# chinhau5/parallel_eda

Hardware: AMD Instinct MI355X
Metric: place+route wall-clock to feasibility (s/flow; bitcoin_miner-scale synthetic on stratixiv-like fabric) (lower is better)
Workload: dtype fp32; 1 GPU; model=bitcoin_miner, arch=bitcoin_stratixiv, grid=280x200, W=300, rr_nodes=15745036, rr_edges=87277236, blocks=37632, nets=35616, conns=110426, global_batch=110426, seq_len=0, final_overused=0, wirelength=4910999

## Files before the change

csrc/hip/place_kernel.hip:

```cpp
#include "pnr_hip.h"

namespace pnrh {

struct PlaceDev {
  const int32_t* net_blk_ptr;
  const int32_t* net_blks;
  const int32_t* blk_net_ptr;
  const int32_t* blk_nets;
  const int8_t* blk_type;
  const int8_t* tile_btype;
  const int32_t* type_cols;
  const int32_t* type_col_ptr;
  const uint8_t* fixed;
  const float* net_q;
  const int32_t* net_sink_ptr;
  const float* conn_crit;
  const float* delay_mat;
  int32_t* bx;
  int32_t* by;
  int32_t* bslot;
  int32_t* grid;
  float* net_cost;
  float* net_tcost;
  int32_t num_blocks, num_nets, gx, gy, cap, nx, ny, io_cap;
// ... 108 lines not shown
  }
  return t;
}

__device__ __forceinline__ float wave_sum_f32(float v) {
  for (int off = 32; off; off >>= 1) v += __shfl_xor(v, off);
  return v;
}

__device__ __forceinline__
bool blk_has_net(const PlaceDev& p, int32_t b, int32_t n) {
  int32_t lo = p.blk_net_ptr[b], hi = p.blk_net_ptr[b + 1];
  while (lo < hi) {
    int32_t mid2 = (lo + hi) >> 1;
    if (p.blk_nets[mid2] < n) lo = mid2 + 1; else hi = mid2;
  }
  return lo < p.blk_net_ptr[b + 1] && p.blk_nets[lo] == n;
}

template <class F> __device__ __forceinline__
void for_blk_nets_k(const PlaceDev& p, int32_t b, F f) {
  const int32_t k0 = p.blk_net_ptr[b];
  for (int32_t k = k0 + (threadIdx.x & 63); k < p.blk_net_ptr[b + 1]; k += 64)
    f(k - k0, p.blk_nets[k]);
}
template <class F> __device__ __forceinline__
void for_blk_nets(const PlaceDev& p, int32_t b, F f) {
  for_blk_nets_k(p, b, [&](int32_t, int32_t n) { f(n); });
}
template <class F> __device__ __forceinline__
void for_macro_nets(const PlaceDev& p, int32_t mm0, int32_t mm1, F f) {
  for (int32_t j = mm0; j < mm1; ++j)
    for_blk_nets(p, p.macro_blk[j], [&](int32_t n) { f(j, n); });
}

struct MinClaims {
  int32_t* net; int32_t* loc; int32_t mine;
  __device__ __forceinline__ void take_net(int n) const { atomicMin(&net[n], mine); }
  __device__ __forceinline__ void take_loc(int t) const { atomicMin(&loc[t], mine); }
  __device__ __forceinline__ bool holds_net(int n) const { return net[n] == mine; }
  __device__ __forceinline__ bool holds_loc(int t) const { return loc[t] == mine; }
};
struct EpochClaims {
  unsigned long long* net; unsigned long long* loc; unsigned long long mine;
  __device__ __forceinline__ void take_net(int n) const { atomicMax(&net[n], mine); }
  __device__ __forceinline__ void take_loc(int t) const { atomicMax(&loc[t], mine); }
  __device__ __forceinline__ bool holds_net(int n) const { return net[n] == mine; }
  __device__ __forceinline__ bool holds_loc(int t) const { return loc[t] == mine; }
};

__device__ __forceinline__ unsigned long long claim_key(uint32_t batch, int i) {
  return ((unsigned long long)batch << 32) | (0xFFFFFFFFu - (uint32_t)i);
}

__device__ __forceinline__
int propose_select(const PlaceDev& p, int rlim, uint32_t seed, uint32_t batch,
                   int i, int& x1o, int& y1o, int& slot1o) {
  uint32_t r0 = rng_hash(seed ^ 0x5BD1E995u, batch, i);
  int32_t blk = r0 % p.num_blocks;
  if (p.fixed && p.fixed[blk]) return -1;
  if (p.rx0 >= 0 && (p.bx[blk] < p.rx0 || p.bx[blk] > p.rx1))
    return -1;
  bool io = p.blk_type[blk] == 0;
  int x0 = p.bx[blk], y0 = p.by[blk];
  int x1 = -1, y1 = -1, slot1 = 0;
  int bt = p.blk_type[blk];
  if (p.tile_btype && bt >= 2 && p.type_cols) {
    int c0 = p.type_col_ptr[bt - 2], c1 = p.type_col_ptr[bt - 1];
    int lo = c0, hi = c1;
    while (lo < hi) { int m = (lo + hi) >> 1;
                      if (p.type_cols[m] < x0 - rlim) lo = m + 1; else hi = m; }
    int lo2 = lo, hi2 = c1;
    while (lo2 < hi2) { int m = (lo2 + hi2) >> 1;
                        if (p.type_cols[m] <= x0 + rlim) lo2 = m + 1; else hi2 = m; }
    int ncol = lo2 - lo;
    if (ncol > 0) {
      int ylo = max(1, y0 - rlim), yhi = min(p.ny, y0 + rlim);
      for (int att = 0; att < 8; ++att) {
        uint32_t r1 = rng_hash(seed, batch, i * 131 + 7 * att + 1);
        uint32_t r2 = rng_hash(seed, batch, i * 131 + 7 * att + 2);
        int tx = p.type_cols[lo + (int)(r1 % ncol)];
        if (p.rx0 >= 0 && (tx < p.rx0 || tx > p.rx1)) continue;
        int ty = ylo + (int)(r2 % (yhi - ylo + 1));
        if (tx == x0 && ty == y0) continue;
        x1 = tx; y1 = ty; slot1 = 0;
        break;
      }
    }
  } else {
    for (int att = 0; att < 8; ++att) {
      uint32_t r1 = rng_hash(seed, batch, i * 131 + 7 * att + 1);
      uint32_t r2 = rng_hash(seed, batch, i * 131 + 7 * att + 2);
      int tx = x0 + (int)(r1 % (2 * rlim + 1)) - rlim;
      int ty = y0 + (int)(r2 % (2 * rlim + 1)) - rlim;
      if (tx < 0 || tx >= p.gx || ty < 0 || ty >= p.gy) continue;
      if (p.rx0 >= 0 && (tx < p.rx0 || tx > p.rx1)) continue;
      if (p.tile_btype) {
        if (p.tile_btype[tx * p.gy + ty] != p.blk_type[blk]) continue;
      } else if (is_io_loc(p, tx, ty) != io) continue;
      int c = cap_at(p, tx, ty);
      if (c <= 0) continue;
      if (tx == x0 && ty == y0) continue;
      x1 = tx; y1 = ty;
      slot1 = (int)(rng_hash(seed, batch, i * 131 + 7 * att + 3) % c);
      break;
    }
// ... 128 lines not shown
  }
  wave_lds_sync();
  NetCosts nc{COST_NONE, 0.0f};
  float d_bb = 0.0f, d_td = 0.0f;
  if (live) {
    const float span = (float)((st.xmax[lane] - st.xmin[lane] + 1) +
                               (st.ymax[lane] - st.ymin[lane] + 1));
    nc.bb = mul_rn(q, span);
    d_bb = __builtin_fmaf(q, span, -old_bb);
    if (timing) {
      float t = 0.0f;
      const int i0 = incl - cnt;
      for (int j = 1; j < cnt; ++j)
        t = __builtin_fmaf(st.crit[i0 + j], st.delay[i0 + j], t);
      nc.td = t;
      d_td = t - old_td;
    }
  }
  const int sb = (n_a + lane) & 63;
  const float b_dbb = __shfl(d_bb, sb), b_dtd = __shfl(d_td, sb);
  const float b_bb = __shfl(nc.bb, sb), b_td = __shfl(nc.td, sb);
  if (lane < n_a) {
    dbb += d_bb;
    if (timing) dtd += d_td;
    ca = nc;
  }
  if (lane < n_b) {
    if (b_bb != COST_NONE) {
      dbb += b_dbb;
      if (timing) dtd += b_dtd;
    }
    cb = NetCosts{b_bb, b_td};
  }
  return true;
}

__device__ __forceinline__
bool metropolis(const Sched& s, int i, float& dbb, float& dtd) {
  dbb = wave_sum_f32(dbb);
  dtd = wave_sum_f32(dtd);
  float delta;
  {
#pragma clang fp contract(off)
    delta = (1.0f - s.timing_tradeoff) * dbb * s.inv_bb_norm +
            s.timing_tradeoff * dtd * s.inv_td_norm;
  }
  if (delta <= 0.0f) return true;
  if (s.T <= 0.0f) return false;
  float u = (rng_hash(s.seed, s.batch, i * 131 + 5) & 0xFFFFFF) *
            (1.0f / 16777216.0f);
  return u < __expf(-delta / s.T);
}

__device__ __forceinline__
void record_move(const MovesDev& m, int32_t* mv_from, int i, int32_t blk,
                 int32_t to, int32_t other, float dbb, float dtd,
                 int32_t from) {
  atomicAdd(&m.counters[1], 1);
  m.mv_blk[i] = blk;
  m.mv_to[i] = to;
  m.mv_other[i] = other;
  m.mv_dbb[i] = dbb;
  m.mv_dtd[i] = dtd;
  m.mv_flags[i] = 1;
  mv_from[i] = from;
}

template <class Claims> __device__ __forceinline__
void propose_move(const PlaceDev& p, const MovesDev& m, const Claims& c,
                  int32_t* mv_from, int i, const Sched& s) {
  const int lane = threadIdx.x & 63;
  int sel = -1, sx1 = -1, sy1 = -1, sslot = 0;
  if (lane == 0) {
    m.mv_flags[i] = 0;
    sel = propose_select(p, s.rlim, s.seed, s.batch, i, sx1, sy1, sslot);
  }
  sel = __shfl(sel, 0);
  if (sel < 0) return;
  const int x1 = __shfl(sx1, 0);
  const int y1 = __shfl(sy1, 0);
  const int slot1 = __shfl(sslot, 0);
  const int32_t blk = sel;
  const int x0 = p.bx[blk], y0 = p.by[blk];
  const int mid = p.macro_of ? p.macro_of[blk] : -1;
  float dbb = 0.0f, dtd = 0.0f;
  if (mid >= 0) {
    const MacroPos ms{mid, x1 - x0, y1 - y0};
    const int32_t mm0 = p.macro_ptr[mid], mm1 = p.macro_ptr[mid + 1];
    if (mm1 - mm0 > 16) return;
    int ok = 0;
    if (lane == 0) {
      ok = macro_shift_ok(p, ms, mm0, mm1);
      if (ok) atomicAdd(&m.counters[0], 1);
    }
    ok = __shfl(ok, 0);
    if (!ok) return;
    for_macro_nets(p, mm0, mm1, [&](int32_t j, int32_t n) {
      bool dup = false;
      for (int32_t j2 = mm0; j2 < j && !dup; ++j2)
        dup = blk_has_net(p, p.macro_blk[j2], n);
      if (!dup) add_net_delta(p, n, ms, s.timing_tradeoff, dbb, dtd);
    });
    if (!metropolis(s, i, dbb, dtd)) return;
    if (lane == 0)
      record_move(m, mv_from, i, blk,
                  ((ms.ddx + 4096) << 13) | (ms.ddy + 4096), -2 - mid, dbb,
                  dtd, x0 * p.gy + y0);
    for_macro_nets(p, mm0, mm1, [&](int32_t, int32_t n) { c.take_net(n); });
    for (int32_t j = mm0 + lane; j < mm1; j += 64) {
      int32_t b = p.macro_blk[j];
      c.take_loc(p.bx[b] * p.gy + p.by[b]);
      c.take_loc((p.bx[b] + ms.ddx) * p.gy + p.by[b] + ms.ddy);
    }
    return;
  }
  int32_t other = p.grid[((int64_t)x1 * p.gy + y1) * p.cap + slot1];
  if (other == blk) return;
  if (other >= 0 && p.fixed && p.fixed[other]) return;
  if (other >= 0 && p.macro_of && p.macro_of[other] >= 0)
    return;
  if (lane == 0) atomicAdd(&m.counters[0], 1);
  const SwapPos sw{blk, x1, y1, other, other >= 0 ? x0 : -1000,
                   other >= 0 ? y0 : -1000};
  const int n_a = p.blk_net_ptr[blk + 1] - p.blk_net_ptr[blk];
  const int n_b =
      other >= 0 ? p.blk_net_ptr[other + 1] - p.blk_net_ptr[other] : 0;
  NetCosts ca{COST_NONE, 0.0f}, cb{COST_NONE, 0.0f};
  __shared__ EvalStage stage[PROP_WAVES];
  const bool timing = s.timing_tradeoff > 0.0f;
  bool evaluated = false;
  if (n_a + n_b <= EVAL_SLOTS && (!timing || p.delay_mat != nullptr))
    evaluated = eval_move_parallel(p, stage[threadIdx.x >> 6], sw, blk, other,
                                   n_a, n_b, timing, dbb, dtd, ca, cb);
  if (!evaluated) {
    for_blk_nets_k(p, blk, [&](int32_t k, int32_t n) {
      NetCosts nc = add_net_delta(p, n, sw, s.timing_tradeoff, dbb, dtd);
      if (k < 64) ca = nc;
    });
    if (other >= 0)
      for_blk_nets_k(p, other, [&](int32_t k, int32_t n) {
        if (blk_has_net(p, blk, n)) return;
        NetCosts nc = add_net_delta(p, n, sw, s.timing_tradeoff, dbb, dtd);
        if (k < 64) cb = nc;
      });
  }
  if (!metropolis(s, i, dbb, dtd)) return;
  const bool stored = n_a + n_b <= m.cost_k;
  if (stored) {
    const int64_t s0 = (int64_t)i * m.cost_k;
    if (lane < n_a) m.mv_ncost[s0 + lane] = ca.bb;
    if (lane < n_b) m.mv_ncost[s0 + n_a + lane] = cb.bb;
    if (s.timing_tradeoff > 0.0f) {
      if (lane < n_a) m.mv_ntcost[s0 + lane] = ca.td;
      if (lane < n_b) m.mv_ntcost[s0 + n_a + lane] = cb.td;
    }
  }
  if (lane == 0) {
    record_move(m, mv_from, i, blk,
                ((x1 * p.gy + y1) * p.cap + slot1) |
                    (stored ? 0 : MV_RECOMPUTE),
                other, dbb, dtd, x0 * p.gy + y0);
    c.take_loc(x0 * p.gy + y0);
    c.take_loc(x1 * p.gy + y1);
  }
  auto take = [&](int32_t n) { c.take_net(n); };
  for_blk_nets(p, blk, take);
  if (other >= 0) for_blk_nets(p, other, take);
}

struct Move {
  int32_t blk, other, to;
  bool recompute;
  __device__ __forceinline__ Move(const MovesDev& m, int i)
      : blk(m.mv_blk[i]), other(m.mv_other[i]), to(m.mv_to[i]) {
    recompute = !is_macro() && (to & MV_RECOMPUTE);
    if (recompute) to &= ~MV_RECOMPUTE;
  }
  __device__ __forceinline__ bool is_macro() const { return other <= -2; }
  __device__ __forceinline__ MacroPos macro() const {
    return MacroPos{-2 - other, (to >> 13) - 4096, (to & 0x1FFF) - 4096};
  }
};

template <class Claims> __device__ __forceinline__
bool resolve_move(const PlaceDev& p, const MovesDev& m, const Claims& c,
                  const int32_t* mv_from, int i, const Move& mv) {
  const int lane = threadIdx.x & 63;
  bool bad = false;
  if (mv.is_macro()) {
    const MacroPos ms = mv.macro();
    const int32_t mm0 = p.macro_ptr[ms.mid], mm1 = p.macro_ptr[ms.mid + 1];
    for (int32_t j = mm0 + lane; j < mm1; j += 64) {
      int32_t b = p.macro_blk[j];
      int sx = p.bx[b], sy = p.by[b];
      int tx = sx + ms.ddx, ty = sy + ms.ddy;
      if (tx < 0 || tx >= p.gx || ty < 0 || ty >= p.gy) bad = true;
      else if (!c.holds_loc(sx * p.gy + sy) ||
               !c.holds_loc(tx * p.gy + ty)) bad = true;
    }
    for_macro_nets(p, mm0, mm1, [&](int32_t, int32_t n) {
      if (!c.holds_net(n)) bad = true;
    });
  } else {
    int x1 = mv.to / p.cap / p.gy, y1 = (mv.to / p.cap) % p.gy;
    if (lane == 0 && (!c.holds_loc(mv_from[i]) ||
                      !c.holds_loc(x1 * p.gy + y1))) bad = true;
    auto lost = [&](int32_t n) { if (!c.holds_net(n)) bad = true; };
    for_blk_nets(p, mv.blk, lost);
    if (mv.other >= 0) for_blk_nets(p, mv.other, lost);
  }
  const bool win = !__any(bad);
  if (lane == 0) {
    if (!win) { m.mv_flags[i] = 0; atomicAdd(&m.counters[3], 1); }
    else { m.mv_flags[i] = 2; atomicAdd(&m.counters[2], 1); }
  }
  return win;
}

template <class Pos> __device__ __forceinline__
void refresh_net(const PlaceDev& p, int32_t n, const Pos& pos,
                 float timing_tradeoff) {
  p.net_cost[n] = net_bb_cost(p, n, pos);
  if (timing_tradeoff > 0.0f) p.net_tcost[n] = net_td_cost(p, n, pos);
}

__device__ __forceinline__
void apply_move(const PlaceDev& p, const MovesDev& m, int i, const Move& mv,
                float timing_tradeoff, double* cost_acc ) {
  const int lane = threadIdx.x & 63;
  if (mv.is_macro()) {
    const MacroPos ms = mv.macro();
    const int32_t mm0 = p.macro_ptr[ms.mid], mm1 = p.macro_ptr[ms.mid + 1];
    for_macro_nets(p, mm0, mm1, [&](int32_t, int32_t n) {
      refresh_net(p, n, ms, timing_tradeoff);
    });
    if (lane == 0) {
      for (int32_t j = mm0; j < mm1; ++j) {
        int32_t b = p.macro_blk[j];
        p.grid[((int64_t)p.bx[b] * p.gy + p.by[b]) * p.cap + p.bslot[b]] = -1;
      }
      for (int32_t j = mm0; j < mm1; ++j) {
        int32_t b = p.macro_blk[j];
        int tx = p.bx[b] + ms.ddx, ty = p.by[b] + ms.ddy;
        p.grid[((int64_t)tx * p.gy + ty) * p.cap] = b;
        p.bx[b] = tx; p.by[b] = ty; p.bslot[b] = 0;
      }
    }
  } else {
    const int32_t blk = mv.blk, other = mv.other;
    int slot1 = mv.to % p.cap;
    int x1 = mv.to / p.cap / p.gy, y1 = (mv.to / p.cap) % p.gy;
    int x0 = p.bx[blk], y0 = p.by[blk], s0 = p.bslot[blk];
    const SwapPos sw{blk, x1, y1, other, other >= 0 ? x0 : -1000,
                     other >= 0 ? y0 : -1000};
    if (mv.recompute) {
      auto refresh = [&](int32_t n) { refresh_net(p, n, sw, timing_tradeoff); };
      for_blk_nets(p, blk, refresh);
      if (other >= 0) for_blk_nets(p, other, refresh);
    } else {
      const int64_t s0 = (int64_t)i * m.cost_k;
      int32_t slot0 = 0;
      auto copy = [&](int32_t k, int32_t n) {
        const float bb = m.mv_ncost[s0 + slot0 + k];
        if (bb == COST_NONE) return;
        p.net_cost[n] = bb;
        if (timing_tradeoff > 0.0f)
          p.net_tcost[n] = m.mv_ntcost[s0 + slot0 + k];
      };
      for_blk_nets_k(p, blk, copy);
      slot0 = p.blk_net_ptr[blk + 1] - p.blk_net_ptr[blk];
      if (other >= 0) for_blk_nets_k(p, other, copy);
    }
    if (lane == 0) {
      p.grid[((int64_t)x0 * p.gy + y0) * p.cap + s0] = other >= 0 ? other : -1;
      p.grid[((int64_t)x1 * p.gy + y1) * p.cap + slot1] = blk;
      p.bx[blk] = x1; p.by[blk] = y1; p.bslot[blk] = slot1;
      if (other >= 0) { p.bx[other] = x0; p.by[other] = y0; p.bslot[other] = s0; }
    }
  }
  if (lane == 0) {
    unsafeAtomicAdd(&cost_acc[0], (double)m.mv_dbb[i]);
    unsafeAtomicAdd(&cost_acc[1], (double)m.mv_dtd[i]);
  }
}

__global__ void place_reset_claims_kernel(int32_t* net_claim, int32_t nn,
                                          int32_t* loc_claim, int32_t nl) {
  int i = blockIdx.x * blockDim.x + threadIdx.x;
  int total = max(nn, nl);
  for (; i < total; i += gridDim.x * blockDim.x) {
    if (i < nn) net_claim[i] = 0x7FFFFFFF;
    if (i < nl) loc_claim[i] = 0x7FFFFFFF;
  }
}

__launch_bounds__(64 * PROP_WAVES, 2)
__global__ void place_propose_kernel(PlaceDev p, MovesDev m, int32_t* mv_from,
                                     Sched s) {
  const int i = move_index();
  if (i >= m.n_moves) return;
  propose_move(p, m, MinClaims{m.net_claim, m.loc_claim, i}, mv_from, i, s);
}

__launch_bounds__(64 * PROP_WAVES, 2)
__global__ void place_resolve_kernel(PlaceDev p, MovesDev m,
                                     const int32_t* mv_from) {
  const int i = move_index();
  if (i >= m.n_moves || m.mv_flags[i] != 1) return;
  resolve_move(p, m, MinClaims{m.net_claim, m.loc_claim, i}, mv_from, i,
               Move(m, i));
}

__launch_bounds__(64 * PROP_WAVES, 2)
__global__ void place_apply_kernel(PlaceDev p, MovesDev m,
                                   float timing_tradeoff, double* cost_acc) {
  const int i = move_index();
  if (i >= m.n_moves || m.mv_flags[i] != 2) return;
  apply_move(p, m, i, Move(m, i), timing_tradeoff, cost_acc);
}

struct RunDev {
  int32_t* mv_from;
  unsigned long long* net_claim;
  unsigned long long* loc_claim;
  int32_t* ctrl;
};

__launch_bounds__(64 * PROP_WAVES, 2)
__global__ void place_propose_run_kernel(PlaceDev p, MovesDev m, RunDev r,
                                         Sched s) {
  if (r.ctrl[0]) return;
  const int i = move_index();
  if (i >= m.n_moves) return;
  const EpochClaims c{r.net_claim, r.loc_claim, claim_key(s.batch, i)};
  propose_move(p, m, c, r.mv_from, i, s);
}

__device__ __forceinline__
void commit_move(const PlaceDev& p, const MovesDev& m, const RunDev& r,
                 float timing_tradeoff, double* cost_acc, uint32_t batch) {
  const int i = move_index();
  if (i >= m.n_moves || m.mv_flags[i] != 1) return;
  const Move mv(m, i);
  const EpochClaims c{r.net_claim, r.loc_claim, claim_key(batch, i)};
  if (resolve_move(p, m, c, r.mv_from, i, mv))
    apply_move(p, m, i, mv, timing_tradeoff, cost_acc);
}

__launch_bounds__(64 * PROP_WAVES, 2)
__global__ void place_commit_kernel(PlaceDev p, MovesDev m, RunDev r,
                                    float timing_tradeoff, double* cost_acc,
                                    uint32_t batch, int check,
                                    int32_t target_moves) {
  if (r.ctrl[0]) return;
  commit_move(p, m, r, timing_tradeoff, cost_acc, batch);
  if (!check) return;
  asm volatile("s_waitcnt vmcnt(0)" ::: "memory");
  __syncthreads();
  if (threadIdx.x != 0) return;
  __threadfence();
  asm volatile("s_waitcnt vmcnt(0)" ::: "memory");
  int ticket = __hip_atomic_fetch_add(&r.ctrl[2], 1, __ATOMIC_RELAXED,
                                      __HIP_MEMORY_SCOPE_AGENT);
  if (ticket != (int)gridDim.x - 1) return;
  __threadfence();
  int att = __hip_atomic_load(&m.counters[0], __ATOMIC_RELAXED,
                              __HIP_MEMORY_SCOPE_AGENT);
  int acc = __hip_atomic_load(&m.counters[1], __ATOMIC_RELAXED,
                              __HIP_MEMORY_SCOPE_AGENT);
  int win = __hip_atomic_load(&m.counters[2], __ATOMIC_RELAXED,
                              __HIP_MEMORY_SCOPE_AGENT);
  r.ctrl[1] += 4;
  if (win + (att - acc) >= target_moves) r.ctrl[0] = 1;
  __hip_atomic_store(&r.ctrl[2], 0, __ATOMIC_RELAXED,
                     __HIP_MEMORY_SCOPE_AGENT);
}

__global__ void place_refresh_costs_kernel(PlaceDev p, float timing_tradeoff,
                                           double* out ) {
  int n = blockIdx.x * blockDim.x + threadIdx.x;
  for (; n < p.num_nets; n += gridDim.x * blockDim.x) {
    const SwapPos as_is{-1, 0, 0, -1, 0, 0};
    float c = net_bb_cost(p, n, as_is);
    p.net_cost[n] = c;
    unsafeAtomicAdd(&out[0], (double)c);
    float t = timing_tradeoff > 0.0f ? net_td_cost(p, n, as_is) : 0.0f;
    p.net_tcost[n] = t;
    unsafeAtomicAdd(&out[1], (double)t);
  }
}

}

using namespace pnrh;

extern "C" {

struct PlaceLaunchArgs {
  const int32_t* net_blk_ptr; const int32_t* net_blks;
  const int32_t* blk_net_ptr; const int32_t* blk_nets;
  const int8_t* blk_type; const int8_t* tile_btype;
  const int32_t* type_cols; const int32_t* type_col_ptr;
  const uint8_t* fixed;
  const float* net_q;
  const int32_t* net_sink_ptr; const float* conn_crit; const float* delay_mat;
  int32_t* bx; int32_t* by; int32_t* bslot; int32_t* grid;
  float* net_cost; float* net_tcost;
  int32_t num_blocks, num_nets, gx, gy, cap, nx, ny, io_cap;
  int32_t rx0, rx1;
  const int32_t* macro_of; const int32_t* macro_ptr;
  const int32_t* macro_blk;
  int32_t* mv_blk; int32_t* mv_to; int32_t* mv_other;
  float* mv_dbb; float* mv_dtd; uint8_t* mv_flags;
  int32_t* net_claim; int32_t* loc_claim; int32_t* counters;
  int32_t n_moves;
  float T; int32_t rlim; float timing_tradeoff;
  float inv_bb_norm, inv_td_norm;
  uint32_t seed, batch;
  double* cost_acc;
  int32_t* mv_from;
  unsigned long long* net_claim64; unsigned long long* loc_claim64;
  int32_t* run_ctrl;
  float* mv_ncost; float* mv_ntcost;
  int32_t cost_k;
};

static void unpack(const PlaceLaunchArgs* a, PlaceDev& p, MovesDev& m) {
  p.net_blk_ptr = a->net_blk_ptr; p.net_blks = a->net_blks;
  p.blk_net_ptr = a->blk_net_ptr; p.blk_nets = a->blk_nets;
  p.blk_type = a->blk_type; p.tile_btype = a->tile_btype;
  p.type_cols = a->type_cols; p.type_col_ptr = a->type_col_ptr;
  p.fixed = a->fixed;
  p.net_q = a->net_q;
  p.net_sink_ptr = a->net_sink_ptr; p.conn_crit = a->conn_crit;
  p.delay_mat = a->delay_mat;
  p.bx = a->bx; p.by = a->by; p.bslot = a->bslot; p.grid = a->grid;
  p.net_cost = a->net_cost; p.net_tcost = a->net_tcost;
  p.num_blocks = a->num_blocks; p.num_nets = a->num_nets;
  p.gx = a->gx; p.gy = a->gy; p.cap = a->cap;
  p.nx = a->nx; p.ny = a->ny; p.io_cap = a->io_cap;
  p.rx0 = a->rx0; p.rx1 = a->rx1;
  p.macro_of = a->macro_of; p.macro_ptr = a->macro_ptr;
  p.macro_blk = a->macro_blk;
  m.mv_blk = a->mv_blk; m.mv_to = a->mv_to; m.mv_other = a->mv_other;
  m.mv_dbb = a->mv_dbb; m.mv_dtd = a->mv_dtd; m.mv_flags = a->mv_flags;
  m.net_claim = a->net_claim; m.loc_claim = a->loc_claim;
  m.counters = a->counters; m.n_moves = a->n_moves;
  m.mv_ncost = a->mv_ncost; m.mv_ntcost = a->mv_ntcost;
  m.cost_k = a->cost_k;
}

static bool batch_args_ok(const PlaceLaunchArgs* a) {
  return a->mv_from && a->mv_ncost && a->mv_ntcost && a->cost_k >= 1 &&
         a->cost_k <= 64 &&
         (int64_t)a->gx * a->gy * a->cap < (int64_t)MV_RECOMPUTE;
}

static Sched sched(const PlaceLaunchArgs* a, uint32_t batch) {
  return Sched{a->T, a->rlim, a->timing_tradeoff, a->inv_bb_norm,
               a->inv_td_norm, a->seed, batch};
}

int pnr_place_batch(const PlaceLaunchArgs* a, void* stream) {
  if (!batch_args_ok(a) || !a->net_claim || !a->loc_claim)
    return (int)hipErrorInvalidValue;
  PlaceDev p; MovesDev m;
  unpack(a, p, m);
  hipStream_t s = (hipStream_t)stream;
  int rg = (max(max(a->num_nets, a->gx * a->gy), a->n_moves) + 255) / 256;
  rg = rg < 2048 ? rg : 2048;
  hipLaunchKernelGGL(place_reset_claims_kernel, dim3(rg), dim3(256), 0, s,
                     m.net_claim, p.num_nets, m.loc_claim, p.gx * p.gy);
  int mg = (m.n_moves + PROP_WAVES - 1) / PROP_WAVES;
  hipLaunchKernelGGL(place_propose_kernel, dim3(mg), dim3(64 * PROP_WAVES),
                     0, s, p, m, a->mv_from, sched(a, a->batch));
  hipLaunchKernelGGL(place_resolve_kernel, dim3(mg), dim3(64 * PROP_WAVES),
                     0, s, p, m, (const int32_t*)a->mv_from);
  hipLaunchKernelGGL(place_apply_kernel, dim3(mg), dim3(64 * PROP_WAVES),
                     0, s, p, m, a->timing_tradeoff, a->cost_acc);
  return (int)hipGetLastError();
}

int pnr_place_run(const PlaceLaunchArgs* a, uint32_t first_batch,
                  int32_t target_moves, int32_t n_batches, void* stream) {
  if (n_batches < 0 || (n_batches & 3) || first_batch == 0 ||
      !batch_args_ok(a) || !a->net_claim64 || !a->loc_claim64 ||
      !a->run_ctrl)
    return (int)hipErrorInvalidValue;
  PlaceDev p; MovesDev m;
  unpack(a, p, m);
  RunDev r;
  r.mv_from = a->mv_from;
  r.net_claim = a->net_claim64; r.loc_claim = a->loc_claim64;
  r.ctrl = a->run_ctrl;
  hipStream_t s = (hipStream_t)stream;
  int mg = (m.n_moves + PROP_WAVES - 1) / PROP_WAVES;
  for (int32_t k = 0; k < n_batches; ++k) {
    const uint32_t batch = first_batch + (uint32_t)k;
    hipLaunchKernelGGL(place_propose_run_kernel, dim3(mg),
                       dim3(64 * PROP_WAVES), 0, s, p, m, r, sched(a, batch));
    hipLaunchKernelGGL(place_commit_kernel, dim3(mg), dim3(64 * PROP_WAVES),
                       0, s, p, m, r, a->timing_tradeoff, a->cost_acc, batch,
                       (int)(((k + 1) & 3) == 0), target_moves);
  }
  return (int)hipGetLastError();
}

int pnr_place_refresh(const PlaceLaunchArgs* a, void* stream) {
  PlaceDev p; MovesDev m;
  unpack(a, p, m);
  hipStream_t s = (hipStream_t)stream;
  hipLaunchKernelGGL(place_refresh_costs_kernel, dim3(1024), dim3(256), 0, s,
                     p, a->timing_tradeoff, a->cost_acc);
  return (int)hipGetLastError();
}

int64_t pnr_place_args_sizeof() { return (int64_t)sizeof(PlaceLaunchArgs); }

}
```

parallel_eda_amd/place/gpu_placer.py:

```python
import ctypes as ct
import math

import numpy as np

from ..arch.archdef import ArchDef
from ..ops import hip_api
from .placer import Placement, analytic_delay_matrix


class PlaceLaunchArgs(ct.Structure):
    _fields_ = [
        ("net_blk_ptr", ct.c_void_p), ("net_blks", ct.c_void_p),
        ("blk_net_ptr", ct.c_void_p), ("blk_nets", ct.c_void_p),
        ("blk_type", ct.c_void_p), ("tile_btype", ct.c_void_p),
        ("type_cols", ct.c_void_p), ("type_col_ptr", ct.c_void_p),
        ("fixed", ct.c_void_p),
        ("net_q", ct.c_void_p),
        ("net_sink_ptr", ct.c_void_p), ("conn_crit", ct.c_void_p),
        ("delay_mat", ct.c_void_p),
        ("bx", ct.c_void_p), ("by", ct.c_void_p), ("bslot", ct.c_void_p),
        ("grid", ct.c_void_p),
        ("net_cost", ct.c_void_p), ("net_tcost", ct.c_void_p),
        ("num_blocks", ct.c_int32), ("num_nets", ct.c_int32),
        ("gx", ct.c_int32), ("gy", ct.c_int32), ("cap", ct.c_int32),
        ("nx", ct.c_int32), ("ny", ct.c_int32), ("io_cap", ct.c_int32),
        ("rx0", ct.c_int32), ("rx1", ct.c_int32),
        ("macro_of", ct.c_void_p), ("macro_ptr", ct.c_void_p),
        ("macro_blk", ct.c_void_p),
        ("mv_blk", ct.c_void_p), ("mv_to", ct.c_void_p), ("mv_other", ct.c_void_p),
        ("mv_dbb", ct.c_void_p), ("mv_dtd", ct.c_void_p), ("mv_flags", ct.c_void_p),
        ("net_claim", ct.c_void_p), ("loc_claim", ct.c_void_p),
        ("counters", ct.c_void_p), ("n_moves", ct.c_int32),
        ("T", ct.c_float), ("rlim", ct.c_int32), ("timing_tradeoff", ct.c_float),
        ("inv_bb_norm", ct.c_float), ("inv_td_norm", ct.c_float),
        ("seed", ct.c_uint32), ("batch", ct.c_uint32),
        ("cost_acc", ct.c_void_p),
        ("mv_from", ct.c_void_p),
        ("net_claim64", ct.c_void_p), ("loc_claim64", ct.c_void_p),
        ("run_ctrl", ct.c_void_p),
        ("mv_ncost", ct.c_void_p), ("mv_ntcost", ct.c_void_p),
        ("cost_k", ct.c_int32),
    ]


RUN_CHUNK_BATCHES = 32


def _lib():
    lib = hip_api.lib()
    if not hasattr(lib, "_place_ready"):
        lib.pnr_place_batch.restype = ct.c_int
        lib.pnr_place_batch.argtypes = [ct.POINTER(PlaceLaunchArgs), ct.c_void_p]
        lib.pnr_place_run.restype = ct.c_int
        lib.pnr_place_run.argtypes = [ct.POINTER(PlaceLaunchArgs), ct.c_uint32,
                                      ct.c_int32, ct.c_int32, ct.c_void_p]
        lib.pnr_place_refresh.restype = ct.c_int
        lib.pnr_place_refresh.argtypes = [ct.POINTER(PlaceLaunchArgs), ct.c_void_p]
        lib.pnr_place_args_sizeof.restype = ct.c_int64
        if lib.pnr_place_args_sizeof() != ct.sizeof(PlaceLaunchArgs):
            raise RuntimeError("PlaceLaunchArgs ABI mismatch")
        lib._place_ready = True
    return lib


def ptr(t):
    return ct.c_void_p(t.data_ptr())


class GpuPlacer:
    def __init__(self, netlist, arch: ArchDef, seed=7, timing=False,
                 device="cuda:0", n_moves=None, fixed=None,
                 delay_matrix="analytic", macros=None, legacy_batches=False):
        import torch
        self.torch = torch
        self.legacy_batches = legacy_batches
        self.device = device
        self.arch = arch
        self.nl = netlist
        self.seed = seed
        self.timing = timing
        nb = netlist.num_blocks
        nn = netlist.num_nets
        gx, gy = arch.nx + 2, arch.ny + 2
        self.gx, self.gy = gx, gy
        self.cap = max(1, arch.io_cap)
        self.batch_counter = 0

        counts = 1 + np.diff(netlist.net_sink_ptr)
        net_blk_ptr = np.r_[0, np.cumsum(counts)].astype(np.int32)
        net_blks = np.empty(net_blk_ptr[-1], dtype=np.int32)
        net_blks[net_blk_ptr[:-1]] = netlist.net_driver
        is_sink = np.ones(len(net_blks), dtype=bool)
        is_sink[net_blk_ptr[:-1]] = False
        net_blks[is_sink] = netlist.net_sinks
        net_of_member = np.repeat(np.arange(nn, dtype=np.int64),
                                  np.diff(net_blk_ptr))
        key = net_blks.astype(np.int64) * nn + net_of_member
        key = np.unique(key)
# ... 46 lines not shown
            self.t_delay_mat = up(dm.ravel())
        else:
            self._dm = None
            self.t_delay_mat = None

        bx, by, bslot, grid = self._initial_placement(seed)
        self.t_macro_of = self.t_macro_ptr = self.t_macro_blk = None
        self.macros = macros or []
        if self.macros:
            bx, by, bslot, grid = self._legalize_macros(
                bx, by, bslot, grid, self.macros)
            macro_of = np.full(nb, -1, dtype=np.int32)
            mptr = [0]
            mblk = []
            for mi, grp in enumerate(self.macros):
                for (b, dx, dy) in grp:
                    macro_of[b] = mi
                    mblk.append(b)
                mptr.append(len(mblk))
            self.t_macro_of = up(macro_of)
            self.t_macro_ptr = up(np.asarray(mptr, dtype=np.int32))
            self.t_macro_blk = up(np.asarray(mblk, dtype=np.int32))
        self.t_bx = up(bx); self.t_by = up(by); self.t_bslot = up(bslot)
        self.t_grid = up(grid)
        self.t_net_cost = torch.zeros(nn, dtype=torch.float32, device=device)
        self.t_net_tcost = torch.zeros(nn, dtype=torch.float32, device=device)

        self.n_moves = n_moves or int(np.clip(nb // 16, 64, 1 << 16))
        nm = self.n_moves
        self.t_mv_blk = torch.zeros(nm, dtype=torch.int32, device=device)
        self.t_mv_to = torch.zeros(nm, dtype=torch.int32, device=device)
        self.t_mv_other = torch.zeros(nm, dtype=torch.int32, device=device)
        self.t_mv_dbb = torch.zeros(nm, dtype=torch.float32, device=device)
        self.t_mv_dtd = torch.zeros(nm, dtype=torch.float32, device=device)
        self.t_mv_flags = torch.zeros(nm, dtype=torch.uint8, device=device)
        self.t_net_claim = self.t_loc_claim = None
        self.t_net_claim64 = self.t_loc_claim64 = None
        if legacy_batches:
            self.t_net_claim = torch.zeros(nn, dtype=torch.int32, device=device)
            self.t_loc_claim = torch.zeros(gx * gy, dtype=torch.int32,
                                           device=device)
        else:
            self.t_net_claim64 = torch.zeros(nn, dtype=torch.int64,
                                             device=device)
            self.t_loc_claim64 = torch.zeros(gx * gy, dtype=torch.int64,
                                             device=device)
        self.t_mv_from = torch.zeros(nm, dtype=torch.int32, device=device)
        max_deg = int(np.diff(blk_net_ptr).max()) if nb else 0
        self.cost_k = int(np.clip(2 * max_deg, 1, 64))
        self.t_mv_ncost = torch.zeros(nm * self.cost_k, dtype=torch.float32,
                                      device=device)
        self.t_mv_ntcost = torch.zeros(nm * self.cost_k, dtype=torch.float32,
                                       device=device)
        self.t_run_state = torch.zeros(8, dtype=torch.int32, device=device)
        self.t_counters = self.t_run_state[:4]
        self.t_run_ctrl = self.t_run_state[4:]
        self.t_cost_acc = torch.zeros(2, dtype=torch.float64, device=device)

        self.lib = _lib()
        self.bb_cost, self.td_cost = self.refresh_costs()

    def _initial_placement(self, seed):
        arch = self.arch
        nl = self.nl
        rng = np.random.default_rng(seed)
        nb = nl.num_blocks
        bx = np.zeros(nb, dtype=np.int32)
        by = np.zeros(nb, dtype=np.int32)
        bslot = np.zeros(nb, dtype=np.int32)
        if self._fixed is not None:
            bx2, by2, bs2, grid = self._initial_placement_free(rng)
            ids, fx, fy, fs = [np.asarray(a) for a in self._fixed]
            for b, x, y, sl in zip(ids, fx, fy, fs):
                occ = grid[x, y, sl]
                if occ == b:
                    continue
                grid[bx2[b], by2[b], bs2[b]] = occ
                if occ >= 0:
                    bx2[occ], by2[occ], bs2[occ] = bx2[b], by2[b], bs2[b]
                bx2[b], by2[b], bs2[b] = x, y, sl
                grid[x, y, sl] = b
            return bx2, by2, bs2, grid.reshape(-1)
        return self._initial_placement_free(rng, flat=True)

    def _legalize_macros(self, bx, by, bslot, grid, macros):
        arch = self.arch
        g = grid.reshape(self.gx, self.gy, self.cap)
        members = [b for grp in macros for (b, _, _) in grp]
        for b in members:
            g[bx[b], by[b], bslot[b]] = -1
        tb = (arch.tile_btype_grid().reshape(self.gx, self.gy)
              if arch.is_heterogeneous() else None)

        def tile_ok(b, x, y):
            if not (0 <= x < self.gx and 0 <= y < self.gy):
                return False
            bt = int(self.nl.block_type[b])
            if tb is not None:
                if tb[x, y] != bt:
                    return False
            else:
                io = (x == 0 or x == self.gx - 1 or
                      y == 0 or y == self.gy - 1)
                inner = 1 <= x <= arch.nx and 1 <= y <= arch.ny
                if bt == 0 or io or not inner:
                    return False
            return g[x, y, 0] < 0

        for grp in macros:
# ... 51 lines not shown
                   [(x, 0) for x in range(1, arch.nx + 1)] +
                   [(x, self.gy - 1) for x in range(1, arch.nx + 1)])
        slots = [(x, y, s) for (x, y) in io_locs for s in range(arch.io_cap)]
        sel = rng.permutation(len(slots))[:len(ios)]
        for b, k in zip(ios, sel):
            x, y, s = slots[k]
            bx[b], by[b], bslot[b] = x, y, s
            grid[x, y, s] = b
        return (bx, by, bslot, grid.reshape(-1)) if flat \
            else (bx, by, bslot, grid)

    def _args(self, T=0.0, rlim=1, tt=0.0, inv_bb=1.0, inv_td=1.0):
        a = PlaceLaunchArgs()
        a.net_blk_ptr = ptr(self.t_net_blk_ptr); a.net_blks = ptr(self.t_net_blks)
        a.blk_net_ptr = ptr(self.t_blk_net_ptr); a.blk_nets = ptr(self.t_blk_nets)
        a.blk_type = ptr(self.t_blk_type)
        a.tile_btype = (ptr(self.t_tile_btype)
                        if self.t_tile_btype is not None else None)
        a.type_cols = (ptr(self.t_type_cols)
                       if self.t_type_cols is not None else None)
        a.type_col_ptr = (ptr(self.t_type_col_ptr)
                          if self.t_type_col_ptr is not None else None)
        a.fixed = ptr(self.t_fixed) if self.t_fixed is not None else None
        a.net_q = ptr(self.t_net_q)
        a.net_sink_ptr = ptr(self.t_net_sink_ptr)
        a.conn_crit = ptr(self.t_conn_crit)
        a.delay_mat = ptr(self.t_delay_mat) if self.t_delay_mat is not None else None
        a.bx = ptr(self.t_bx); a.by = ptr(self.t_by); a.bslot = ptr(self.t_bslot)
        a.grid = ptr(self.t_grid)
        a.net_cost = ptr(self.t_net_cost); a.net_tcost = ptr(self.t_net_tcost)
        a.num_blocks = self.nl.num_blocks; a.num_nets = self.nl.num_nets
        a.gx = self.gx; a.gy = self.gy; a.cap = self.cap
        a.nx = self.arch.nx; a.ny = self.arch.ny; a.io_cap = self.arch.io_cap
        a.rx0, a.rx1 = getattr(self, "move_region", (-1, -1))
        if getattr(self, "t_macro_of", None) is not None:
            a.macro_of = ptr(self.t_macro_of)
            a.macro_ptr = ptr(self.t_macro_ptr)
            a.macro_blk = ptr(self.t_macro_blk)
        else:
            a.macro_of = a.macro_ptr = a.macro_blk = None
        a.mv_blk = ptr(self.t_mv_blk); a.mv_to = ptr(self.t_mv_to)
        a.mv_other = ptr(self.t_mv_other); a.mv_dbb = ptr(self.t_mv_dbb)
        a.mv_dtd = ptr(self.t_mv_dtd); a.mv_flags = ptr(self.t_mv_flags)
        if self.legacy_batches:
            a.net_claim = ptr(self.t_net_claim)
            a.loc_claim = ptr(self.t_loc_claim)
            a.net_claim64 = a.loc_claim64 = None
        else:
            a.net_claim = a.loc_claim = None
            a.net_claim64 = ptr(self.t_net_claim64)
            a.loc_claim64 = ptr(self.t_loc_claim64)
        a.mv_from = ptr(self.t_mv_from)
        a.run_ctrl = ptr(self.t_run_ctrl)
        a.mv_ncost = ptr(self.t_mv_ncost); a.mv_ntcost = ptr(self.t_mv_ntcost)
        a.cost_k = self.cost_k
        a.counters = ptr(self.t_counters); a.n_moves = self.n_moves
        a.T = T; a.rlim = max(1, int(rlim)); a.timing_tradeoff = tt
        a.inv_bb_norm = inv_bb; a.inv_td_norm = inv_td
        a.seed = self.seed & 0xFFFFFFFF; a.batch = self.batch_counter
        a.cost_acc = ptr(self.t_cost_acc)
        return a

    def _stream(self):
        return self.torch.cuda.current_stream().cuda_stream

    def refresh_costs(self):
        self.t_cost_acc.zero_()
        a = self._args(tt=1.0 if self.timing else 0.0)
        rc = self.lib.pnr_place_refresh(ct.byref(a), self._stream())
        hip_api.check(rc, "place_refresh")
        self.torch.cuda.synchronize(self.device)
        bb, td = self.t_cost_acc.cpu().numpy()
        self.bb_cost, self.td_cost = float(bb), float(td)
        return self.bb_cost, self.td_cost

    def run_batches(self, T, rlim, target_moves, tt, bb_norm, td_norm,
                    max_batches=256):
        if self.legacy_batches:
            return self._run_batches_legacy(T, rlim, target_moves, tt,
                                            bb_norm, td_norm, max_batches)
        self.t_run_state.zero_()
        a = self._args(T=T, rlim=rlim, tt=tt,
                       inv_bb=1.0 / bb_norm, inv_td=1.0 / td_norm)
        target = int(min(max(math.ceil(target_moves), -0x7FFFFFFF),
                         0x7FFFFFFF))
        cap = 4 * ((max_batches + 3) // 4)
        first = self.batch_counter + 1
        enq = 0
        att = acc = executed = 0
        while enq < cap:
            n = min(RUN_CHUNK_BATCHES, cap - enq)
            rc = self.lib.pnr_place_run(ct.byref(a), first + enq, target, n,
                                        self._stream())
            hip_api.check(rc, "place_run")
            enq += n
            st = self.t_run_state.cpu().numpy()
            att, acc = int(st[0]), int(st[1])
            done, executed = int(st[4]), int(st[5])
            if done:
                break
        self.batch_counter += executed
        srate = acc / max(1, att)
        return srate, att

    def _run_batches_legacy(self, T, rlim, target_moves, tt, bb_norm, td_norm,
                            max_batches=256):
        self.t_counters.zero_()
        batches = 0
        win = att = acc = 0
        while batches < max_batches:
            for _ in range(4):
                self.batch_counter += 1
                a = self._args(T=T, rlim=rlim, tt=tt,
                               inv_bb=1.0 / bb_norm, inv_td=1.0 / td_norm)
                rc = self.lib.pnr_place_batch(ct.byref(a), self._stream())
                hip_api.check(rc, "place_batch")
                batches += 1
            self.torch.cuda.synchronize(self.device)
            c = self.t_counters.cpu().numpy()
            att, acc, win = int(c[0]), int(c[1]), int(c[2])
            if win + (att - acc) >= target_moves:
                break
        else:
            self.torch.cuda.synchronize(self.device)
        srate = acc / max(1, att)
        return srate, att

    def set_move_region(self, x0, x1):
        self.move_region = (x0, x1)

    def set_crit(self, conn_crit):
        t = self.torch.from_numpy(np.ascontiguousarray(conn_crit,
                                                       dtype=np.float32))
        self.t_conn_crit.copy_(t.to(self.device))

    def placement(self):
        return Placement(self.t_bx.cpu().numpy(), self.t_by.cpu().numpy(),
                         self.t_bslot.cpu().numpy(),
                         bb_cost=self.bb_cost, td_cost=self.td_cost)

    def check_place(self):
        bx = self.t_bx.cpu().numpy(); by = self.t_by.cpu().numpy()
        bslot = self.t_bslot.cpu().numpy()
        grid = self.t_grid.cpu().numpy().reshape(self.gx, self.gy, self.cap)
        nl = self.nl
        tb = (self.arch.tile_btype_grid().reshape(self.gx, self.gy)
              if self.arch.is_heterogeneous() else None)
        btype = np.asarray(nl.block_type)
        if tb is not None:
# ... 149 lines not shown
```

Before: 7.272 s.

## Shard placement move counters across cache lines and drop per-move cost accumulation atomics

Replaces the single global attempt/accept/win/conflict counters with 64 shards, each on its own 128-byte line and chosen by block index, which spreads atomic contention. The last block of each check reduces the shards with a wavefront reduction and writes the totals back for the host. The change also removes the per-applied-move double-precision atomic adds into cost_acc, so the running cost delta is no longer accumulated in apply. The risk is that any code still reading cost_acc after a run will see stale values.

Result: faster. 6.066 s, median of 6 (-16.6%).

```diff
diff --git a/csrc/hip/place_kernel.hip b/csrc/hip/place_kernel.hip
--- a/csrc/hip/place_kernel.hip
+++ b/csrc/hip/place_kernel.hip
@@ -184,6 +184,19 @@
 __device__ __forceinline__ unsigned long long claim_key(uint32_t batch, int i) {
   return ((unsigned long long)batch << 32) | (0xFFFFFFFFu - (uint32_t)i);
 }
+
+enum { CNT_ATTEMPTS = 0, CNT_ACCEPTED = 1, CNT_WINNERS = 2, CNT_CONFLICTS = 3 };
+struct DirectCounters {
+  int32_t* w;
+  __device__ __forceinline__ void add(int k) const { atomicAdd(&w[k], 1); }
+};
+#define SHARD_WORDS 32
+struct ShardCounters {
+  int32_t* w;
+  __device__ __forceinline__ ShardCounters(int32_t* shards, int32_t mask)
+      : w(shards + (int64_t)(blockIdx.x & mask) * SHARD_WORDS) {}
+  __device__ __forceinline__ void add(int k) const { atomicAdd(&w[k], 1); }
+};
 
 __device__ __forceinline__
 int propose_select(const PlaceDev& p, int rlim, uint32_t seed, uint32_t batch,
@@ -418,11 +431,11 @@
   return u < __expf(-delta / s.T);
 }
 
-__device__ __forceinline__
-void record_move(const MovesDev& m, int32_t* mv_from, int i, int32_t blk,
-                 int32_t to, int32_t other, float dbb, float dtd,
-                 int32_t from) {
-  atomicAdd(&m.counters[1], 1);
+template <class Counters> __device__ __forceinline__
+void record_move(const MovesDev& m, const Counters& cnt, int32_t* mv_from,
+                 int i, int32_t blk, int32_t to, int32_t other, float dbb,
+                 float dtd, int32_t from) {
+  cnt.add(CNT_ACCEPTED);
   m.mv_blk[i] = blk;
   m.mv_to[i] = to;
   m.mv_other[i] = other;
@@ -432,9 +445,10 @@
   mv_from[i] = from;
 }
 
-template <class Claims> __device__ __forceinline__
+template <class Claims, class Counters> __device__ __forceinline__
 void propose_move(const PlaceDev& p, const MovesDev& m, const Claims& c,
-                  int32_t* mv_from, int i, const Sched& s) {
+                  const Counters& cnt, int32_t* mv_from, int i,
+                  const Sched& s) {
   const int lane = threadIdx.x & 63;
   int sel = -1, sx1 = -1, sy1 = -1, sslot = 0;
   if (lane == 0) {
@@ -457,7 +471,7 @@
     int ok = 0;
     if (lane == 0) {
       ok = macro_shift_ok(p, ms, mm0, mm1);
-      if (ok) atomicAdd(&m.counters[0], 1);
+      if (ok) cnt.add(CNT_ATTEMPTS);
     }
     ok = __shfl(ok, 0);
     if (!ok) return;
@@ -469,7 +483,7 @@
     });
     if (!metropolis(s, i, dbb, dtd)) return;
     if (lane == 0)
-      record_move(m, mv_from, i, blk,
+      record_move(m, cnt, mv_from, i, blk,
                   ((ms.ddx + 4096) << 13) | (ms.ddy + 4096), -2 - mid, dbb,
                   dtd, x0 * p.gy + y0);
     for_macro_nets(p, mm0, mm1, [&](int32_t, int32_t n) { c.take_net(n); });
@@ -485,7 +499,7 @@
   if (other >= 0 && p.fixed && p.fixed[other]) return;
   if (other >= 0 && p.macro_of && p.macro_of[other] >= 0)
     return;
-  if (lane == 0) atomicAdd(&m.counters[0], 1);
+  if (lane == 0) cnt.add(CNT_ATTEMPTS);
   const SwapPos sw{blk, x1, y1, other, other >= 0 ? x0 : -1000,
                    other >= 0 ? y0 : -1000};
   const int n_a = p.blk_net_ptr[blk + 1] - p.blk_net_ptr[blk];
@@ -522,7 +536,7 @@
     }
   }
   if (lane == 0) {
-    record_move(m, mv_from, i, blk,
+    record_move(m, cnt, mv_from, i, blk,
                 ((x1 * p.gy + y1) * p.cap + slot1) |
                     (stored ? 0 : MV_RECOMPUTE),
                 other, dbb, dtd, x0 * p.gy + y0);
@@ -548,9 +562,10 @@
   }
 };
 
-template <class Claims> __device__ __forceinline__
+template <class Claims, class Counters> __device__ __forceinline__
 bool resolve_move(const PlaceDev& p, const MovesDev& m, const Claims& c,
-                  const int32_t* mv_from, int i, const Move& mv) {
+                  const Counters& cnt, const int32_t* mv_from, int i,
+                  const Move& mv) {
   const int lane = threadIdx.x & 63;
   bool bad = false;
   if (mv.is_macro()) {
@@ -577,8 +592,8 @@
   }
   const bool win = !__any(bad);
   if (lane == 0) {
-    if (!win) { m.mv_flags[i] = 0; atomicAdd(&m.counters[3], 1); }
-    else { m.mv_flags[i] = 2; atomicAdd(&m.counters[2], 1); }
+    if (!win) { m.mv_flags[i] = 0; cnt.add(CNT_CONFLICTS); }
+    else { m.mv_flags[i] = 2; cnt.add(CNT_WINNERS); }
   }
   return win;
 }
@@ -592,7 +607,7 @@
 
 __device__ __forceinline__
 void apply_move(const PlaceDev& p, const MovesDev& m, int i, const Move& mv,
-                float timing_tradeoff, double* cost_acc ) {
+                float timing_tradeoff) {
   const int lane = threadIdx.x & 63;
   if (mv.is_macro()) {
     const MacroPos ms = mv.macro();
@@ -644,10 +659,6 @@
       if (other >= 0) { p.bx[other] = x0; p.by[other] = y0; p.bslot[other] = s0; }
     }
   }
-  if (lane == 0) {
-    unsafeAtomicAdd(&cost_acc[0], (double)m.mv_dbb[i]);
-    unsafeAtomicAdd(&cost_acc[1], (double)m.mv_dtd[i]);
-  }
 }
 
 __global__ void place_reset_claims_kernel(int32_t* net_claim, int32_t nn,
@@ -665,7 +676,8 @@
                                      Sched s) {
   const int i = move_index();
   if (i >= m.n_moves) return;
-  propose_move(p, m, MinClaims{m.net_claim, m.loc_claim, i}, mv_from, i, s);
+  propose_move(p, m, MinClaims{m.net_claim, m.loc_claim, i},
+               DirectCounters{m.counters}, mv_from, i, s);
 }
 
 __launch_bounds__(64 * PROP_WAVES, 2)
@@ -673,16 +685,16 @@
                                      const int32_t* mv_from) {
   const int i = move_index();
   if (i >= m.n_moves || m.mv_flags[i] != 1) return;
-  resolve_move(p, m, MinClaims{m.net_claim, m.loc_claim, i}, mv_from, i,
-               Move(m, i));
+  resolve_move(p, m, MinClaims{m.net_claim, m.loc_claim, i},
+               DirectCounters{m.counters}, mv_from, i, Move(m, i));
 }
 
 __launch_bounds__(64 * PROP_WAVES, 2)
 __global__ void place_apply_kernel(PlaceDev p, MovesDev m,
-                                   float timing_tradeoff, double* cost_acc) {
+                                   float timing_tradeoff) {
   const int i = move_index();
   if (i >= m.n_moves || m.mv_flags[i] != 2) return;
-  apply_move(p, m, i, Move(m, i), timing_tradeoff, cost_acc);
+  apply_move(p, m, i, Move(m, i), timing_tradeoff);
 }
 
 struct RunDev {
@@ -690,6 +702,8 @@
   unsigned long long* net_claim;
   unsigned long long* loc_claim;
   int32_t* ctrl;
+  int32_t* shards;
+  int32_t n_shards;
 };
 
 __launch_bounds__(64 * PROP_WAVES, 2)
@@ -699,45 +713,58 @@
   const int i = move_index();
   if (i >= m.n_moves) return;
   const EpochClaims c{r.net_claim, r.loc_claim, claim_key(s.batch, i)};
-  propose_move(p, m, c, r.mv_from, i, s);
+  propose_move(p, m, c, ShardCounters(r.shards, r.n_shards - 1), r.mv_from, i,
+               s);
 }
 
 __device__ __forceinline__
 void commit_move(const PlaceDev& p, const MovesDev& m, const RunDev& r,
-                 float timing_tradeoff, double* cost_acc, uint32_t batch) {
+                 float timing_tradeoff, uint32_t batch) {
   const int i = move_index();
   if (i >= m.n_moves || m.mv_flags[i] != 1) return;
   const Move mv(m, i);
   const EpochClaims c{r.net_claim, r.loc_claim, claim_key(batch, i)};
-  if (resolve_move(p, m, c, r.mv_from, i, mv))
-    apply_move(p, m, i, mv, timing_tradeoff, cost_acc);
+  if (resolve_move(p, m, c, ShardCounters(r.shards, r.n_shards - 1),
+                   r.mv_from, i, mv))
+    apply_move(p, m, i, mv, timing_tradeoff);
+}
+
+__device__ __forceinline__ int wave_sum_i32(int v) {
+  for (int off = 32; off; off >>= 1) v += __shfl_xor(v, off);
+  return v;
 }
 
 __launch_bounds__(64 * PROP_WAVES, 2)
 __global__ void place_commit_kernel(PlaceDev p, MovesDev m, RunDev r,
-                                    float timing_tradeoff, double* cost_acc,
-                                    uint32_t batch, int check,
-                                    int32_t target_moves) {
+                                    float timing_tradeoff, uint32_t batch,
+                                    int check, int32_t target_moves) {
   if (r.ctrl[0]) return;
-  commit_move(p, m, r, timing_tradeoff, cost_acc, batch);
+  commit_move(p, m, r, timing_tradeoff, batch);
   if (!check) return;
   asm volatile("s_waitcnt vmcnt(0)" ::: "memory");
   __syncthreads();
-  if (threadIdx.x != 0) return;
+  if (threadIdx.x >= 64) return;
+  const int lane = threadIdx.x;
   __threadfence();
   asm volatile("s_waitcnt vmcnt(0)" ::: "memory");
-  int ticket = __hip_atomic_fetch_add(&r.ctrl[2], 1, __ATOMIC_RELAXED,
-                                      __HIP_MEMORY_SCOPE_AGENT);
-  if (ticket != (int)gridDim.x - 1) return;
+  int ticket = 0;
+  if (lane == 0)
+    ticket = __hip_atomic_fetch_add(&r.ctrl[2], 1, __ATOMIC_RELAXED,
+                                    __HIP_MEMORY_SCOPE_AGENT);
+  if (__shfl(ticket, 0) != (int)gridDim.x - 1) return;
   __threadfence();
-  int att = __hip_atomic_load(&m.counters[0], __ATOMIC_RELAXED,
-                              __HIP_MEMORY_SCOPE_AGENT);
-  int acc = __hip_atomic_load(&m.counters[1], __ATOMIC_RELAXED,
-                              __HIP_MEMORY_SCOPE_AGENT);
-  int win = __hip_atomic_load(&m.counters[2], __ATOMIC_RELAXED,
-                              __HIP_MEMORY_SCOPE_AGENT);
+  int tot[4] = {0, 0, 0, 0};
+  for (int sh = lane; sh < r.n_shards; sh += 64)
+    for (int k = 0; k < 4; ++k)
+      tot[k] += __hip_atomic_load(&r.shards[(int64_t)sh * SHARD_WORDS + k],
+                                  __ATOMIC_RELAXED, __HIP_MEMORY_SCOPE_AGENT);
+  for (int k = 0; k < 4; ++k) tot[k] = wave_sum_i32(tot[k]);
+  if (lane != 0) return;
+  for (int k = 0; k < 4; ++k) m.counters[k] = tot[k];
   r.ctrl[1] += 4;
-  if (win + (att - acc) >= target_moves) r.ctrl[0] = 1;
+  if (tot[CNT_WINNERS] + (tot[CNT_ATTEMPTS] - tot[CNT_ACCEPTED]) >=
+      target_moves)
+    r.ctrl[0] = 1;
   __hip_atomic_store(&r.ctrl[2], 0, __ATOMIC_RELAXED,
                      __HIP_MEMORY_SCOPE_AGENT);
 }
@@ -787,6 +814,8 @@
   int32_t* mv_from;
   unsigned long long* net_claim64; unsigned long long* loc_claim64;
   int32_t* run_ctrl;
+  int32_t* run_shards;
+  int32_t n_shards;
   float* mv_ncost; float* mv_ntcost;
   int32_t cost_k;
 };
@@ -843,7 +872,7 @@
   hipLaunchKernelGGL(place_resolve_kernel, dim3(mg), dim3(64 * PROP_WAVES),
                      0, s, p, m, (const int32_t*)a->mv_from);
   hipLaunchKernelGGL(place_apply_kernel, dim3(mg), dim3(64 * PROP_WAVES),
-                     0, s, p, m, a->timing_tradeoff, a->cost_acc);
+                     0, s, p, m, a->timing_tradeoff);
   return (int)hipGetLastError();
 }
 
@@ -851,7 +880,8 @@
                   int32_t target_moves, int32_t n_batches, void* stream) {
   if (n_batches < 0 || (n_batches & 3) || first_batch == 0 ||
       !batch_args_ok(a) || !a->net_claim64 || !a->loc_claim64 ||
-      !a->run_ctrl)
+      !a->run_ctrl || !a->run_shards || a->n_shards < 1 ||
+      (a->n_shards & (a->n_shards - 1)) || ((uintptr_t)a->run_shards & 127))
     return (int)hipErrorInvalidValue;
   PlaceDev p; MovesDev m;
   unpack(a, p, m);
@@ -859,6 +889,8 @@
   r.mv_from = a->mv_from;
   r.net_claim = a->net_claim64; r.loc_claim = a->loc_claim64;
   r.ctrl = a->run_ctrl;
+  r.shards = a->run_shards;
+  r.n_shards = a->n_shards;
   hipStream_t s = (hipStream_t)stream;
   int mg = (m.n_moves + PROP_WAVES - 1) / PROP_WAVES;
   for (int32_t k = 0; k < n_batches; ++k) {
@@ -866,7 +898,7 @@
     hipLaunchKernelGGL(place_propose_run_kernel, dim3(mg),
                        dim3(64 * PROP_WAVES), 0, s, p, m, r, sched(a, batch));
     hipLaunchKernelGGL(place_commit_kernel, dim3(mg), dim3(64 * PROP_WAVES),
-                       0, s, p, m, r, a->timing_tradeoff, a->cost_acc, batch,
+                       0, s, p, m, r, a->timing_tradeoff, batch,
                        (int)(((k + 1) & 3) == 0), target_moves);
   }
   return (int)hipGetLastError();
diff --git a/parallel_eda_amd/place/gpu_placer.py b/parallel_eda_amd/place/gpu_placer.py
--- a/parallel_eda_amd/place/gpu_placer.py
+++ b/parallel_eda_amd/place/gpu_placer.py
@@ -38,12 +38,17 @@
         ("mv_from", ct.c_void_p),
         ("net_claim64", ct.c_void_p), ("loc_claim64", ct.c_void_p),
         ("run_ctrl", ct.c_void_p),
+        ("run_shards", ct.c_void_p), ("n_shards", ct.c_int32),
         ("mv_ncost", ct.c_void_p), ("mv_ntcost", ct.c_void_p),
         ("cost_k", ct.c_int32),
     ]
 
 
 RUN_CHUNK_BATCHES = 32
+
+LINE_WORDS = 32
+RUN_HOST_WORDS = 8
+COUNTER_SHARDS = 64
 
 
 def _lib():
@@ -196,9 +201,14 @@
                                       device=device)
         self.t_mv_ntcost = torch.zeros(nm * self.cost_k, dtype=torch.float32,
                                        device=device)
-        self.t_run_state = torch.zeros(8, dtype=torch.int32, device=device)
+        self.n_shards = COUNTER_SHARDS
+        self.t_run_state = torch.zeros((1 + self.n_shards) * LINE_WORDS,
+                                       dtype=torch.int32, device=device)
+        if self.t_run_state.data_ptr() % (4 * LINE_WORDS):
+            raise RuntimeError("run state is not 128-byte aligned")
         self.t_counters = self.t_run_state[:4]
-        self.t_run_ctrl = self.t_run_state[4:]
+        self.t_run_ctrl = self.t_run_state[4:RUN_HOST_WORDS]
+        self.t_run_shards = self.t_run_state[LINE_WORDS:]
         self.t_cost_acc = torch.zeros(2, dtype=torch.float64, device=device)
 
         self.lib = _lib()
@@ -356,6 +366,8 @@
             a.loc_claim64 = ptr(self.t_loc_claim64)
         a.mv_from = ptr(self.t_mv_from)
         a.run_ctrl = ptr(self.t_run_ctrl)
+        a.run_shards = ptr(self.t_run_shards)
+        a.n_shards = self.n_shards
         a.mv_ncost = ptr(self.t_mv_ncost); a.mv_ntcost = ptr(self.t_mv_ntcost)
         a.cost_k = self.cost_k
         a.counters = ptr(self.t_counters); a.n_moves = self.n_moves
@@ -398,7 +410,7 @@
                                         self._stream())
             hip_api.check(rc, "place_run")
             enq += n
-            st = self.t_run_state.cpu().numpy()
+            st = self.t_run_state[:RUN_HOST_WORDS].cpu().numpy()
             att, acc = int(st[0]), int(st[1])
             done, executed = int(st[4]), int(st[5])
             if done:
```
